# yml-bit/CTA-GAN

Measured on AMD Instinct MI355X. Metric: paired 512x512 slices/sec (G+D step); generator rel-L2 vs CPU reference, higher is better.
Workload: dtype bf16; 1 GPU; HdGan stage-2 full G+D train step (G, Reg, STN, D_m, losses, Adam x3), 16 paired 512x512 slices/GPU; per_gpu_batch=16, global_batch=16, size=512, parallelism=single, rccl_ranks=1, dp_backend=none

## Files before the change

### cta_gan_amd/csrc/conv_halo.h

```cpp
#pragma once
#include <stdlib.h>
#include <type_traits>
#include "common.h"
#include "conv_dispatch.h"

struct ConvArgs {
    const void* x;
    const void* w;
    void* y;
    const float* bias;
    int B, Hi, Wi, Cin, x_ld;
    int Ho, Wo, Cout, y_ld;
    int Hs, Ws, oy0, ox0, os, is;
    int frame;
    int pad_mode, act;
    int w_tap_stride;
    int ntaps;
    int taps[64];
    int kh, kw, dy0, dx0;
    float* stats;
    const void* res;
    const void* fold;
    int res_ld, fold_ld;
    const void* bz;
    const float* bmean;
    const float* brstd;
    float* bstats;
    int bz_ld, bact;
    int ncls;
    int s2d;
    int pair_lo;
    unsigned long long* nie_sync;
    int nie_act;
    int nie_budget;
    int c_ntaps[4], c_tap0[4], c_oy0[4], c_ox0[4], c_kh[4], c_kw[4], c_dy0[4], c_dx0[4];
};

typedef const __attribute__((address_space(1))) void* gptr_t;
typedef __attribute__((address_space(3))) void* lptr_t;

extern __device__ __attribute__((aligned(16))) unsigned g_zero_chunk[4];

__device__ __forceinline__ void unpack_bf16x8(const u32x4 t, float (&f)[8]) {
#pragma unroll
    for (int i = 0; i < 4; ++i) {
        f[2 * i] = __uint_as_float(t[i] << 16);
        f[2 * i + 1] = __uint_as_float(t[i] & 0xffff0000u);
    }
}
__device__ __forceinline__ void add_bf16x8(float (&f)[8], const bf16_t* p) {
    const u32x4 t = *reinterpret_cast<const u32x4*>(p);
#pragma unroll
    for (int i = 0; i < 4; ++i) {
        f[2 * i] += __uint_as_float(t[i] << 16);
        f[2 * i + 1] += __uint_as_float(t[i] & 0xffff0000u);
    }
}

#define HALO_W 16

template <typename T, typename OutT, int BN, int WM, int WN, int KCH, int ABUF, int TH, bool FUSE, int KWC, bool MC = false, bool PK = false,
          bool S2D = false, bool NIE = false>
__global__ __launch_bounds__(WM * WN * 64, ((TH / WM) * (BN / (WN * 16)) > 16 ? 2 : 4))
void conv_halo_kernel(const ConvArgs a) {
    static_assert(!NIE || (!MC && !S2D && sizeof(T) == 2 && !std::is_same<OutT, float>::value),
                  "InstanceNorm in the epilogue: plain bf16 / split-pair launches");
    static_assert(!S2D || (!MC && !FUSE && KWC == 0 && ABUF == 1), "polyphase K walk: plain single-buffer instantiations");
    static_assert(!PK || (KCH == 8 && sizeof(T) == 2), "split-pair K steps: [hi 32 | lo 32] rows of bf16");
    constexpr int NTH = WM * WN * 64;
    constexpr int EPC = VecOf<T>::N;
    constexpr int BKE = KCH * EPC;
    constexpr int BM = TH * HALO_W;
    constexpr int TM = TH / WM;
    static_assert(TH % WM == 0, "tile rows per wave");
    constexpr int TN = BN / (WN * 16);
    constexpr int B_CH = BN * KCH;
    constexpr int B_IT = (B_CH + NTH - 1) / NTH;
    static_assert(B_CH % 64 == 0, "weight tile");
    extern __shared__ __attribute__((aligned(16))) char smem[];

    const int tid = threadIdx.x, lane = tid & 63, wave = __builtin_amdgcn_readfirstlane(tid >> 6);
    const int wm = wave / WN, wn = wave % WN;
    const int n = blockIdx.y;
// ... 8 lines not shown
        kh_ = a.c_kh[q]; kw_ = a.c_kw[q]; dy0 = a.c_dy0[q]; dx0 = a.c_dx0[q];
        ntaps = a.c_ntaps[q]; tap0 = a.c_tap0[q]; oy0_ = a.c_oy0[q]; ox0_ = a.c_ox0[q];
    }
    const int HPW = KWC ? HALO_W + KWC - 1 : HALO_W + kw_ - 1, HPH = TH + kh_ - 1;
    const int HPC = HPH * HPW * KCH;
    const int HPC64 = (HPC + 63) & ~63;
    const int nchunk = a.Cin / BKE;
    const int nbufA = (nchunk > 1 && ABUF == 2) ? 2 : 1;
    char* sA = smem;
    char* sB = smem + nbufA * HPC64 * 16;

    const int tx_n = (a.Ws + HALO_W - 1) / HALO_W;
    const int y0 = (sp / tx_n) * TH, x0 = (sp % tx_n) * HALO_W;
    const T* __restrict__ X = (const T*)a.x + (size_t)n * a.Hi * a.Wi * a.x_ld;
    const T* __restrict__ W = (const T*)a.w;

    const int h_it = (HPC64 + NTH - 1) / NTH;
    const unsigned hpw_magic = (unsigned)((0x100000000ULL + HPW - 1) / HPW);
    const int Hi = a.Hi, Wi = a.Wi, x_ld = a.x_ld, pad_mode = a.pad_mode;
    const int iy00 = y0 + dy0, ix00 = x0 + dx0;
    constexpr bool PRE = (KWC >= 3) && !MC;
    constexpr int H_PRE = PRE ? ((((TH + KWC - 1) * (HALO_W + KWC - 1) * KCH + 63) & ~63) + NTH - 1) / NTH : 1;
    int hoff[H_PRE];
    if constexpr (PRE) {
#pragma unroll
        for (int it = 0; it < H_PRE; ++it) {
            const int sl = tid + NTH * it;
            const int hrow = sl / KCH;
            const int hy = (int)__umulhi((unsigned)hrow, hpw_magic), hx = hrow - hy * HPW;
            const int kc = swz<KCH>(hx, sl % KCH);
// ... 110 lines not shown
#pragma unroll
            for (int mt = 0; mt < TM; ++mt)
#pragma unroll
                for (int nt = 0; nt < TN; ++nt) {
                    if constexpr (sizeof(T) == 2) {
                        acc[mt][nt] = __builtin_amdgcn_mfma_f32_16x16x32_bf16(
                            __builtin_bit_cast(bf16x8, fb[nt]), __builtin_bit_cast(bf16x8, fa[mt]), acc[mt][nt], 0, 0, 0);
                    } else {
                        const f32x4 va = __builtin_bit_cast(f32x4, fa[mt]);
                        const f32x4 vb = __builtin_bit_cast(f32x4, fb[nt]);
#pragma unroll
                        for (int q = 0; q < 4; ++q)
                            acc[mt][nt] = __builtin_amdgcn_mfma_f32_16x16x4f32(vb[q], va[q], acc[mt][nt], 0, 0, 0);
                    }
                }
        }
    };

    const bool wave_rows_valid = y0 + wm * TM < a.Hs;
    const int pps = (h_it + ntaps - 1) / ntaps;
    auto issue_halo_all = [&](int buf, int kc0) __attribute__((always_inline)) {
        if constexpr (PRE) {
#pragma unroll
            for (int j = 0; j < H_PRE; ++j)
                if (NTH * j + 64 * wave < HPC64) {
                    const T* src = hoff[j] >= 0 ? X + (hoff[j] + kc0) : (const T*)g_zero_chunk;
                    __builtin_amdgcn_global_load_lds((gptr_t)src, (lptr_t)(sA + (buf * HPC64 + NTH * j + 64 * wave) * 16), 16, 0, 0);
                }
        } else {
            for (int it = 0; it < h_it; ++it) issue_halo(it, buf, kc0);
// ... 369 lines not shown
        __syncthreads();
#pragma unroll
        for (int it = 0; it < NIT; ++it) {
            const int cidx = tid + NTH * it;
            const int prow = cidx / CPR, ch = (cidx % CPR) * 8;
            const int oy = y0 + prow / HALO_W, ox = x0 + prow % HALO_W;
            if (oy < a.Hs && ox < a.Ws && n0 + ch < a.Cout) {
                OutT* yp = Y + (((size_t)n * a.Ho + (oy * a.os + oy0_)) * a.Wo + (ox * a.os + ox0_)) * a.y_ld + n0 + ch;
                u32x4 v = *reinterpret_cast<const u32x4*>(st + prow * RS + ch * 2);
                if constexpr (FUSE) {
                    float f[8], g[8];
                    unpack_bf16x8(v, f);
                    unpack_bf16x8(rv[it], g);
#pragma unroll
                    for (int e = 0; e < 8; ++e) f[e] += g[e];
                    if (F != nullptr) {
                        const int ey = oy == 1 ? 0 : (oy == a.Hs - 2 ? a.Hs + 1 : -1);
                        const int ex = ox == 1 ? 0 : (ox == a.Ws - 2 ? a.Ws + 1 : -1);
                        const OutT* Fn = F + (size_t)n * (a.Hs + 2) * (a.Ws + 2) * a.fold_ld + n0 + ch;
                        if (ey >= 0) add_bf16x8(f, Fn + ((size_t)ey * (a.Ws + 2) + ox + 1) * a.fold_ld);
                        if (ex >= 0) add_bf16x8(f, Fn + ((size_t)(oy + 1) * (a.Ws + 2) + ex) * a.fold_ld);
                        if (ey >= 0 && ex >= 0) add_bf16x8(f, Fn + ((size_t)ey * (a.Ws + 2) + ex) * a.fold_ld);
                    }
                    bf16x8 o;
#pragma unroll
                    for (int e = 0; e < 8; ++e) o[e] = (bf16_t)f[e];
                    v = __builtin_bit_cast(u32x4, o);
                    if (bst) {
                        float zf[8];
                        unpack_bf16x8(zv[it], zf);
// ... 71 lines not shown
                    }
                }
                if (vec_ok) {
                    *reinterpret_cast<f32x4*>(yp + co) = f32x4{v[0], v[1], v[2], v[3]};
                } else {
#pragma unroll
                    for (int r = 0; r < 4; ++r)
                        if (co + r < a.Cout) yp[co + r] = v[r];
                }
            }
        }
    }
}

template <typename T, typename OutT, int BN, int WM, int WN, int KCH, int ABUF, int TH = 16, bool FUSE = false, int KWC = 0, bool MC = false, bool PK = false,
          bool S2D = false, bool NIE = false>
static int launch_halo_cfg(const ConvArgs& a, hipStream_t st, int* tiles_out = nullptr) {
    if constexpr (!NIE && KWC == 3 && (TH == 16 || (TH == 8 && !PK)) && BN == 128 && WM == 4 && WN == 2 && KCH == 8 && !MC && !S2D &&
                  sizeof(T) == 2 && ((std::is_same<OutT, bf16_t>::value && !PK) || (std::is_same<OutT, bfpair_t>::value && PK))) {
        if (a.nie_sync != nullptr) {
            if ((FUSE && (a.fold != nullptr || a.bstats != nullptr)) || a.stats == nullptr || a.Cout % BN) return CTG_EINVAL;
            return launch_halo_cfg<T, OutT, BN, WM, WN, KCH, ABUF, TH, FUSE, KWC, false, PK, false, true>(a, st, tiles_out);
        }
    }
    if constexpr (!S2D && !FUSE && !MC && KWC == 0 && TH == 16 && sizeof(T) == 2 && KCH == 8 && BN >= 64 && !std::is_same<OutT, float>::value) {
        if (a.s2d) {
            if (a.res != nullptr || a.fold != nullptr) return -1;
            return launch_halo_cfg<T, OutT, BN, WM, WN, KCH, ABUF, TH, false, 0, false, PK, true>(a, st, tiles_out);
        }
    }
    if (a.s2d && !S2D) return -1;
    if constexpr (!FUSE && !MC && !S2D && !NIE) {
        if (a.res != nullptr || a.fold != nullptr) return launch_halo_cfg<T, OutT, BN, WM, WN, KCH, ABUF, TH, true, KWC, false, PK>(a, st, tiles_out);
    }
    if constexpr (!MC && !S2D && !FUSE && KWC == 0 && (TH == 16 || (TH == 8 && BN == 64)) && sizeof(T) == 2 &&
                  ((std::is_same<OutT, bf16_t>::value && !PK) || (std::is_same<OutT, bfpair_t>::value && PK))) {
        if (a.ncls == 4) return launch_halo_cfg<T, OutT, BN, WM, WN, KCH, ABUF, TH, false, 0, true, PK>(a, st, tiles_out);
    }
    if constexpr (KWC == 0 && !MC && !S2D && sizeof(T) == 2) {
        if (a.kw == 3 && a.kh <= 3 && a.ncls <= 1) return launch_halo_cfg<T, OutT, BN, WM, WN, KCH, ABUF, TH, FUSE, 3, false, PK>(a, st, tiles_out);
    }
    if (a.ncls > 1 && !MC && !S2D) return -1;
    if (a.nie_sync != nullptr && !NIE) return CTG_EINVAL;
    constexpr int NTH = WM * WN * 64;
    const int hpw = HALO_W + a.kw - 1, hph = TH + a.kh - 1;
    const int hpc = hph * hpw * KCH;
    const int hpc64 = (hpc + 63) & ~63;
    const int epc = VecOf<T>::N;
    const int nchunk = a.Cin / (KCH * epc);
    const int main_lds = (((nchunk > 1 && ABUF == 2) ? 2 : 1) * hpc64 + 2 * BN * KCH) * 16;
    const int epi_lds = std::is_same<OutT, bfpair_t>::value ? TH * HALO_W * ((BN / WN) * 4 + 16)
                        : sizeof(OutT) == 2 ? TH * HALO_W * (BN * 2 + 16) : 0;
    if (FUSE && a.bstats != nullptr && WM * WN * 64 * 64 > (main_lds > epi_lds ? main_lds : epi_lds)) return -1;
    const int smem = main_lds > epi_lds ? main_lds : epi_lds;
    if (smem > 160 * 1024 || hph * hpw >= 65536) return -1;
    static unsigned long long attr_mask = 0;
    {
        const int rc = ctg_lds_attr_once((const void*)conv_halo_kernel<T, OutT, BN, WM, WN, KCH, ABUF, TH, FUSE, KWC, MC, PK, S2D, NIE>,
                                         160 * 1024, &attr_mask);
        if (rc != CTG_OK) return rc;
    }
    const int tiles = ((a.Hs + TH - 1) / TH) * ((a.Ws + HALO_W - 1) / HALO_W) * (MC ? 4 : 1);
    if (tiles_out != nullptr) *tiles_out = tiles;
    const int ntn = (a.Cout + BN - 1) / BN;
    if constexpr (NIE) {
        static int occ_dev[64];
        int dev = 0;
        if (hipGetDevice(&dev) != hipSuccess) dev = 0;
        dev &= 63;
        if (occ_dev[dev] == 0) {
            int occ = 0;
            if (hipOccupancyMaxActiveBlocksPerMultiprocessor(
                    &occ, (const void*)conv_halo_kernel<T, OutT, BN, WM, WN, KCH, ABUF, TH, FUSE, KWC, MC, PK, S2D, NIE>, NTH, smem) != hipSuccess ||
                occ < 1)
                occ = 1;
            occ_dev[dev] = occ;
        }
        const int share = ctg_knobs().nie_share > 0 ? ctg_knobs().nie_share : 2;
        if ((long)tiles * ntn * share > (long)occ_dev[dev] * ctg_cu_count()) return 2;
    }
    dim3 grid(tiles * ntn, a.B);
    hipLaunchKernelGGL((conv_halo_kernel<T, OutT, BN, WM, WN, KCH, ABUF, TH, FUSE, KWC, MC, PK, S2D, NIE>), grid, dim3(NTH), smem, st, a);
    return ctg_launch_status();
}

static int launch_strip32(const ConvArgs& a, hipStream_t st, int* tiles_out, bool pair);

template <typename T, int KCH>
static int launch_halo_t(const ConvArgs& a, int out_f32, hipStream_t st, int* tiles_out) {
    if (a.is != 1 && !a.s2d) return -1;
    if (out_f32 >= 2) {
        if constexpr (sizeof(T) == 2 && KCH == 8) {
            if (out_f32 == 2) {
                if (a.Cout > 64) return launch_halo_cfg<T, bfpair_t, 128, 4, 2, 8, 1, 16, false, 0, false, true>(a, st, tiles_out);
                if (a.Cout > 32) {
                    if (a.ncls == 4 && !ctg_knobs().no_mc_th8) return launch_halo_cfg<T, bfpair_t, 64, 4, 1, 8, 1, 8, false, 0, false, true>(a, st, tiles_out);
                    if (!ctg_knobs().no_th8_64 && a.ncls <= 1 && a.Hs >= 16)
// ... 53 lines not shown
```

### cta_gan_amd/csrc/conv_igemm.hip

```cpp
#include <stdlib.h>
#include "conv_halo.h"
#include "conv_strip.h"
#include "conv_stript.h"
#include "conv_pair_strips.h"
#include "conv_strips2.h"
#include "conv_strips2w.h"

__device__ __attribute__((aligned(16))) unsigned g_zero_chunk[4];

#ifndef CTG_BIG_TILE
#define CTG_BIG_TILE 1
#endif
static inline int gather_bm(bool bf16, bool k8, int omode, int Cout, long pixels) {
    return (bf16 && k8 && omode == 0 && Cout > 64 && pixels >= 4096 && CTG_BIG_TILE && !ctg_knobs().no_big_tile) ? 256 : 128;
}

#define FRAME_EDGE_PAD 128
__device__ __forceinline__ void grid_pixel(const ConvArgs& a, int m, int& j, int& i) {
    if (a.frame) {
        const int l1 = a.Hs - 2;
        const int p0 = (a.Ws + FRAME_EDGE_PAD - 1) & ~(FRAME_EDGE_PAD - 1), p1 = (l1 + FRAME_EDGE_PAD - 1) & ~(FRAME_EDGE_PAD - 1);
        if (m < p0) { j = 0; i = m < a.Ws ? m : a.Ws - 1; }
        else if (m < 2 * p0) { j = a.Hs - 1; i = m - p0 < a.Ws ? m - p0 : a.Ws - 1; }
        else {
// ... 473 lines not shown
        return launch_cfg<T, T, 128, 32, 4, 1, KCH, 2>(a, st);
    }
    if (out_f32 || sizeof(T) == 4) return launch_cfg<T, float, 128, 16, 4, 1, KCH, 2>(a, st);
    return CTG_EINVAL;
}

extern "C" int ctg_conv_igemm(int dtype, int out_f32, const void* x, const void* w, void* y, const float* bias,
                              int B, int Hi, int Wi, int Cin, int x_ld, int Ho, int Wo, int Cout, int y_ld,
                              int Hs, int Ws, int oy0, int ox0, int os, int is, int frame, int pad_mode, int act,
                              int w_npad, int ntaps, const int* taps_host, float* stats_part, int* stats_slabs_out,
                              const ctg_conv_epilogue* epi, void* stream) {
    CTG_ENTER();
    const void* res = epi ? epi->res : nullptr;
    const void* fold = epi ? epi->fold : nullptr;
    const int res_ld = epi ? epi->res_ld : 0, fold_ld = epi ? epi->fold_ld : 0;
    if (ntaps < 1 || ntaps > 64 || B < 1 || Hs < 1 || Ws < 1 || Cout < 1) return CTG_EINVAL;
    if (frame != 0 && (frame != 1 || Hs < 3 || Ws < 3)) return CTG_EINVAL;
    if (frame != 0 && stats_part != nullptr) return CTG_EINVAL;
    if (dtype != DT_F32 && dtype != DT_BF16 && dtype != DT_PAIR) return CTG_EINVAL;
    const bool pair = dtype == DT_PAIR;
    if (pair) {
        if (x_ld % 16 != 0 || x_ld < 2 * Cin || Cin % 32 != 0 || (out_f32 != 0 && out_f32 != 1)) return CTG_EINVAL;
        if (!out_f32 && (y_ld % 16 != 0 || y_ld < 2 * Cout || Cout % 8 != 0 || ((uintptr_t)y & 15))) return CTG_EINVAL;
        dtype = DT_BF16;
    } else if (out_f32 != 0 && out_f32 != 1) return CTG_EINVAL;
    const int omode = pair ? (out_f32 ? 3 : 2) : out_f32;
    const int epc = dtype == DT_BF16 ? 8 : 4;
    if (Cin % (4 * epc) != 0 || x_ld % epc != 0 || x_ld < Cin || y_ld < Cout) return CTG_EINVAL;
    if (((uintptr_t)x & 15) || ((uintptr_t)w & 15)) return CTG_EINVAL;
    const bool narrow_out = out_f32 || dtype == DT_F32;
    if (!narrow_out && (Cout % 8 != 0 || y_ld % 8 != 0 || ((uintptr_t)y & 15))) return CTG_EINVAL;
    const int bn = Cout > 64 ? 128 : Cout > 32 ? 64 : Cout > 16 ? 32 : 16;
    if (w_npad < ((Cout + bn - 1) / bn) * bn) return CTG_EINVAL;
    if ((Hs - 1) * os + oy0 >= Ho || (Ws - 1) * os + ox0 >= Wo) return CTG_EINVAL;
    if (stats_slabs_out != nullptr) *stats_slabs_out = 0;
    const bool fused = res != nullptr || fold != nullptr;
    if (fused) {
        if (os != 1 || is != 1 || frame || oy0 || ox0 || Ho != Hs || Wo != Ws || Hs < 4 || Ws < 4 || (out_f32 && Cout <= 16)) return CTG_EINVAL;
        if (res != nullptr && (res_ld < Cout || res_ld % epc || ((uintptr_t)res & 15))) return CTG_EINVAL;
        if (fold != nullptr && (fold_ld < Cout || fold_ld % epc || ((uintptr_t)fold & 15))) return CTG_EINVAL;
    }
    ConvArgs a;
    a.stats = nullptr;
    a.ncls = 1;
    a.nie_sync = nullptr; a.nie_act = ACT_NONE; a.nie_budget = 0;
    a.res = res; a.fold = fold; a.res_ld = res_ld; a.fold_ld = fold_ld;
    a.bz = nullptr; a.bmean = nullptr; a.brstd = nullptr; a.bstats = nullptr; a.bz_ld = 0; a.bact = ACT_NONE;
    if (epi != nullptr && epi->bstats != nullptr) {
        if (!fused || dtype != DT_BF16 || (pair && out_f32) || epi->bz == nullptr || epi->bmean == nullptr || epi->brstd == nullptr ||
            epi->bz_ld < Cout || epi->bz_ld % 8 || ((uintptr_t)epi->bz & 15) || Cout <= 16) return CTG_EINVAL;
        if (epi->bact != ACT_NONE && epi->bact != ACT_RELU && epi->bact != ACT_LRELU) return CTG_EINVAL;
        a.bz = epi->bz; a.bmean = epi->bmean; a.brstd = epi->brstd; a.bstats = epi->bstats; a.bz_ld = epi->bz_ld;
        a.bact = epi->bact;
    }
    a.x = x; a.w = w; a.y = y; a.bias = bias;
    a.B = B; a.Hi = Hi; a.Wi = Wi; a.Cin = Cin; a.x_ld = x_ld;
    a.Ho = Ho; a.Wo = Wo; a.Cout = Cout; a.y_ld = y_ld;
    a.Hs = Hs; a.Ws = Ws; a.oy0 = oy0; a.ox0 = ox0; a.os = os; a.is = is; a.frame = frame;
    a.pad_mode = pad_mode; a.act = act; a.w_tap_stride = w_npad * Cin; a.ntaps = ntaps;
    a.pair_lo = 0;
    const bool k8 = pair || (Cin % (8 * epc)) == 0;
// ... 89 lines not shown
            int ntile = 0;
            const bool want_stats = stats_part != nullptr && stats_slabs_out != nullptr && bias == nullptr &&
                                    act == ACT_NONE && Cout > 16 &&
                                    ((os == 1 && Hs == Ho && Ws == Wo) || os == 2);
            a.stats = want_stats ? stats_part : nullptr;
            int rc = -1;
            if (dtype == DT_BF16) rc = k8 ? launch_halo_t<bf16_t, 8>(a, omode, st, &ntile) : launch_halo_t<bf16_t, 4>(a, omode, st, &ntile);
            else rc = k8 ? launch_halo_t<float, 8>(a, omode, st, &ntile) : launch_halo_t<float, 4>(a, omode, st, &ntile);
            if (rc != -1) {
                if ((want_stats || a.bstats != nullptr) && rc == 0 && stats_slabs_out != nullptr) *stats_slabs_out = ntile;
                return rc;
            }
            a.stats = nullptr;
        }
    }
    if (fused) return CTG_EINVAL;
    if (dtype == DT_BF16 && !out_f32 && !pair) {
        const bool ws = stats_part != nullptr && stats_slabs_out != nullptr;
        int slabs = 0;
        int rc = launch_strips2(a, ws ? stats_part : nullptr, st, &slabs);
        if (rc == -1) rc = launch_strips2w(a, ws ? stats_part : nullptr, st, &slabs);
        if (rc != -1) {
            if (rc == 0 && ws) *stats_slabs_out = slabs;
            return rc;
        }
    }
    int mtiles = 0;
    if (stats_part != nullptr && stats_slabs_out != nullptr && bias == nullptr && act == ACT_NONE &&
        Cout > 16 && os == 1 && !frame && Hs == Ho && Ws == Wo && oy0 == 0 && ox0 == 0) {
        const int bm = gather_bm(dtype == DT_BF16, k8, omode, Cout, (long)Hs * Ws);
// ... 17 lines not shown
                                      void* stream) {
    CTG_ENTER();
    if (stats_slabs_out != nullptr) *stats_slabs_out = 0;
    if (dtype != DT_BF16 && dtype != DT_PAIR) return 2;
    const bool pair = dtype == DT_PAIR;
    if (B < 1 || Hs < 1 || Ws < 1 || Cout < 1 || cls_ntaps == nullptr || cls_oy0 == nullptr || cls_ox0 == nullptr) return CTG_EINVAL;
    if (Cin % 32 != 0 || x_ld % 8 != 0 || x_ld < Cin || y_ld < Cout || Cout % 8 != 0 || y_ld % 8 != 0) return CTG_EINVAL;
    if (pair && (x_ld % 16 || x_ld < 2 * Cin || y_ld % 16 || y_ld < 2 * Cout)) return CTG_EINVAL;
    if (((uintptr_t)x & 15) || ((uintptr_t)w & 15) || ((uintptr_t)y & 15)) return CTG_EINVAL;
    const int bn = Cout > 64 ? 128 : Cout > 32 ? 64 : Cout > 16 ? 32 : 16;
    if (w_npad < ((Cout + bn - 1) / bn) * bn) return CTG_EINVAL;
    if (ctg_knobs().no_halo || ctg_knobs().no_class_merge || Hs < 16 || Ws < 16 || Cout <= 16 || (long)Hi * Wi * x_ld >= (1L << 31)) return 2;
    ConvArgs a;
    a.stats = nullptr;
    a.nie_sync = nullptr; a.nie_act = ACT_NONE; a.nie_budget = 0;
    a.res = nullptr; a.fold = nullptr; a.res_ld = 0; a.fold_ld = 0;
    a.bz = nullptr; a.bmean = nullptr; a.brstd = nullptr; a.bstats = nullptr; a.bz_ld = 0; a.bact = ACT_NONE;
    a.x = x; a.w = w; a.y = y; a.bias = bias;
    a.B = B; a.Hi = Hi; a.Wi = Wi; a.Cin = Cin; a.x_ld = x_ld;
    a.Ho = Ho; a.Wo = Wo; a.Cout = Cout; a.y_ld = y_ld;
    a.Hs = Hs; a.Ws = Ws; a.oy0 = 0; a.ox0 = 0; a.os = 2; a.is = 1; a.frame = 0;
    a.pad_mode = pad_mode; a.act = act; a.w_tap_stride = w_npad * Cin;
    a.ncls = 4;
    a.s2d = 0;
    a.pair_lo = 0;
    if (pair) {
        a.pair_lo = x_ld / 2;
        a.Cin = 2 * Cin;
        a.w_tap_stride = w_npad * 2 * Cin;
    }
    int t0 = 0, kh_max = 1, kw_max = 1;
// ... 37 lines not shown
```

### cta_gan_amd/csrc/conv_strip.h

```cpp
#pragma once
#include "conv_halo.h"

#define STRIP_R 9
#define STRIP_ROWB 1152

struct StripArgs {
    const bf16_t* x;
    const bf16_t* w;
    bf16_t* y;
    const float* bias;
    float* stats;
    int B, H, W, x_ld, y_ld, w_tap_stride;
    int pad_mode, act;
    int band_rows, nbands, nstrips;
    int widx[9];
    int x_lo, y_lo;
};

__device__ __forceinline__ int strip_swz(int px, int c) { return c ^ ((px >> 1) & 3); }

template <bool FLIP, bool EPI>
__global__ __launch_bounds__(256, 2) void conv_strip32_kernel(const StripArgs a) {
    __shared__ __attribute__((aligned(16))) char ring_all[4][STRIP_R][STRIP_ROWB];
    const int tid = threadIdx.x, lane = tid & 63, wave = __builtin_amdgcn_readfirstlane(tid >> 6);
// ... 339 lines not shown
#pragma unroll
            for (int r = 0; r < 4; ++r) {
                const float t1 = row16_sum_to_lane15(s1[nt][r]), t2 = row16_sum_to_lane15(s2[nt][r]);
                if (p == 15) {
                    const int c = nt * 16 + kg * 4 + r;
                    dst[c * 2] = t1;
                    dst[c * 2 + 1] = t2;
                }
            }
    }
}

static int launch_strip32(const ConvArgs& a, hipStream_t st, int* tiles_out, bool pair) {
    if (ctg_knobs().no_strip || a.Cin != (pair ? 64 : 32) || a.Cout != 32 || a.kh != 3 || a.kw != 3 || a.ntaps != 9 || a.is != 1 || a.os != 1 || a.ncls > 1 ||
        a.oy0 != 0 || a.ox0 != 0 || a.Ho != a.Hs || a.Wo != a.Ws || a.Hi != a.Hs || a.Wi != a.Ws || a.res != nullptr ||
        a.fold != nullptr || a.dy0 != -1 || a.dx0 != -1 || a.act > ACT_LRELU)
        return -1;
    if ((long)a.B * a.Hs * a.Ws < (1L << 20) || a.Hs < 32 || a.Ws < 32 || (a.y_ld & 3) || (a.x_ld & 7)) return -1;
    if (pair && (long)a.Hs * a.Ws * a.x_ld >= (1L << 31)) return -1;
    const bool fwd = taps_3x3(a.taps, false);
    if (!fwd && !taps_3x3(a.taps, true)) return -1;
    StripArgs s;
    s.x = (const bf16_t*)a.x; s.w = (const bf16_t*)a.w; s.y = (bf16_t*)a.y; s.bias = a.bias; s.stats = a.stats;
    s.B = a.B; s.H = a.Hs; s.W = a.Ws; s.x_ld = a.x_ld; s.y_ld = a.y_ld; s.w_tap_stride = a.w_tap_stride;
    s.pad_mode = a.pad_mode; s.act = a.act;
    s.x_lo = a.pair_lo; s.y_lo = a.y_ld / 2;
    s.nstrips = (a.Ws + 15) / 16;
    const BandPlan bp = band_plan(a.Hs, 32, (long)ctg_cu_count() * 4 * (pair ? 2 : 3), (long)a.B * s.nstrips, ctg_knobs().strip_band);
    s.band_rows = bp.band_rows;
    s.nbands = bp.nbands;
    for (int t = 0; t < 9; ++t) s.widx[t] = a.taps[t] >> 16;
// ... 25 lines not shown
```

### cta_gan_amd/engine.py

```python
from __future__ import annotations

import os

from dataclasses import dataclass
from typing import Callable, List, Optional

import torch

from . import dp, ops
from .ops import ACT_LRELU, ACT_NONE, ACT_RELU, ACT_SIGMOID, ACT_TANH, PAD_REFLECT, PAD_ZERO, pack_tap


class Act:
    __slots__ = ("t", "grad", "req", "moments", "in_src", "in_plain", "grad_stats")

    def __init__(self, t: torch.Tensor, req: bool = False):
        self.t = t
        self.grad = None
        self.req = req
        self.moments = None
        self.in_src = None
        self.in_plain = False
        self.grad_stats = None

# ... 388 lines not shown
                weight.detach()[0].flip(-1, -2).reshape(cin, kk).contiguous(), _pack_dtype(dtype), 1, cin, kk, _round_up(cin, 32), 64,
                kk, 1, 0))
        dxp = ops.empty_act((bsz, hi + 2 * p, wi + 2 * p, cin), dtype, dev)
        ops.conv_smallcin(g.reshape(bsz, ho, wo), None, spec.k, 1, 2 * p, PAD_ZERO, wflip, _round_up(cin, 32), None,
                          ACT_NONE, dxp, cin, kxw=kxw)
        add_grad(x, dxp, p)
        return
    wb, npad = _pack_bwd(cache, spec, weight, dtype, kpad=m_c if spec.out_f32 else None)
    if spec.transposed:
        dx = ops.empty_act((bsz, hi, wi, cin), dtype, dev)
        taps = [pack_tap(ky - spec.pad, kx - spec.pad, ky * spec.k + kx) for ky in range(spec.k) for kx in range(spec.k)]
        ops.conv_igemm(gm, wb, npad, dx, None, cin, hi, wi, 0, 0, 1, 2, PAD_ZERO, ACT_NONE, taps)
        add_grad(x, dx, 0)
    elif spec.reflect:
        p = spec.pad
        dxp = ops.empty_act((bsz, hi + 2 * p, wi + 2 * p, cin), dtype, dev)
        assert spec.stride == 1
        taps = [pack_tap(-ky, -kx, ky * spec.k + kx) for ky in range(spec.k) for kx in range(spec.k)]
        if p == 1 and hi % 16 == 0 and wi % 16 == 0 and hi >= 32 and wi >= 32 and not _NO_FRAME:
            taps_in = [pack_tap(p - ky, p - kx, ky * spec.k + kx) for ky in range(spec.k) for kx in range(spec.k)]
            if ops.conv_fusable(cin, hi, wi):
                ops.conv_igemm(gm, wb, npad, dxp, None, cin, hi + 2 * p, wi + 2 * p, 0, 0, 1, 1, PAD_ZERO, ACT_NONE, taps,
                               frame=True)
                res = None
                if x.grad is not None and x.grad[1] == 0 and x.grad[0].dtype == dtype \
                        and tuple(x.grad[0].shape) == (bsz, hi, wi, cin):
                    res, x.grad = x.grad[0], None
                dx = ops.empty_act((bsz, hi, wi, cin), dtype, dev)
                want_in = (x.in_src is not None and x.grad is None and dtype == torch.bfloat16 and not _NO_IN_FUSE)
                in_arg = x.in_src if want_in else None
                if want_in and ops.PAIR_BWD_ACTIVE:
                    zact = x.in_src[3]
                    if zact == ACT_RELU and x.in_plain:
                        in_arg = (x.t, _unit_stats(x.t, 0.0), _unit_stats(x.t, 1.0), ACT_RELU)
                    elif zact != ACT_NONE:
                        want_in, in_arg = False, None
                part, slabs = ops.conv_igemm(gm, wb, npad, dx, None, cin, hi, wi, 0, 0, 1, 1, PAD_ZERO, ACT_NONE, taps_in,
                                             res=res, fold=dxp, in_bwd=in_arg)
                add_grad(x, dx, 0)
                if want_in and slabs > 0:
                    x.grad_stats = (dx, part)
                return
            ops.conv_igemm(gm, wb, npad, dxp, None, cin, hi, wi, p, p, 1, 1, PAD_ZERO, ACT_NONE, taps_in)
            ops.conv_igemm(gm, wb, npad, dxp, None, cin, hi + 2 * p, wi + 2 * p, 0, 0, 1, 1, PAD_ZERO, ACT_NONE, taps,
                           frame=True)
        else:
            ops.conv_igemm(gm, wb, npad, dxp, None, cin, hi + 2 * p, wi + 2 * p, 0, 0, 1, 1, PAD_ZERO, ACT_NONE, taps)
        add_grad(x, dxp, p)
    else:
        dx = ops.empty_act((bsz, hi, wi, cin), dtype, dev)
        _bwd_data_launch(spec, gm, wb, npad, dx, hi, wi, cin)
        add_grad(x, dx, 0)


_UNIT_STATS = {}


def _unit_stats(t, value):
    key = (t.device, t.shape[0], t.shape[3], value)
    hit = _UNIT_STATS.get(key)
    if hit is None:
# ... 224 lines not shown
```

### cta_gan_amd/ops.py

```python
from __future__ import annotations

import ctypes
import os
import threading
from typing import Optional, Sequence

import torch

from . import _lib

ACT_NONE, ACT_RELU, ACT_LRELU, ACT_TANH, ACT_SIGMOID = 0, 1, 2, 3, 4
PAD_ZERO, PAD_REFLECT = 0, 1
_DT = {torch.float32: 0, torch.bfloat16: 1}
_EPC = {torch.float32: 4, torch.bfloat16: 8}


def dt(dtype) -> int:
    return _DT[dtype]


def epc(dtype) -> int:
    return _EPC[dtype]


DT_PAIR = 2
DT_MIX = 3

_env = os.environ.get
_NO_NIE = bool(_env("CTG_NO_NIE"))
NIE_POISON = bool(_env("CTG_NIE_POISON"))
NIE_MAX_WGS = int(_env("CTG_NIE_MAX_WGS", "1024"))
NIE_MAX_WGS_PAIR = int(_env("CTG_NIE_MAX_WGS_PAIR", "2048"))
NIE_BUDGET = int(_env("CTG_NIE_BUDGET", "0"))
NIE_SHARE = max(1, int(_env("CTG_NIE_SHARE", "2") or 2))
_TH8_WGS = 0 if _env("CTG_NO_TH8") is not None else int(_env("CTG_TH8_WGS", "384"))
_NO_HALO = bool(_env("CTG_NO_HALO"))
_NO_EPI_FUSE = bool(_env("CTG_NO_EPI_FUSE"))
_NO_WG_GROUPS_FIX = bool(_env("CTG_NO_WG_GROUPS_FIX"))
_WG_S2_FIX = not _env("CTG_NO_WG_S2_FIX")
_WG_FIX_BELOW = int(_env("CTG_WG_FIX_BELOW", "512"))
_NO_SMALLB = bool(_env("CTG_NO_SMALLB"))
_FIN_FUSE = bool(_env("CTG_FIN_FUSE"))
_NO_KXW = bool(_env("CTG_NO_KXW"))
DETERMINISTIC = bool(_env("CTG_DETERMINISTIC"))


def dtc(t) -> int:
    if _pair_now() and t.dtype == torch.bfloat16:
        return DT_PAIR
    return _DT[t.dtype]


# ... 198 lines not shown


def pack_tap(dy: int, dx: int, widx: int) -> int:
    assert -64 <= dy < 64 and -64 <= dx < 64 and 0 <= widx < 256
    return (dy + 64) | ((dx + 64) << 8) | (widx << 16)


def _tap_array(taps: Sequence[int]):
    return (ctypes.c_int * len(taps))(*taps)


class ConvEpilogue(ctypes.Structure):
    _fields_ = [("res", ctypes.c_void_p), ("fold", ctypes.c_void_p), ("bz", ctypes.c_void_p), ("bmean", ctypes.c_void_p),
                ("brstd", ctypes.c_void_p), ("bstats", ctypes.c_void_p), ("res_ld", ctypes.c_int), ("fold_ld", ctypes.c_int),
                ("bz_ld", ctypes.c_int), ("bact", ctypes.c_int), ("nie_sync", ctypes.c_void_p), ("nie_act", ctypes.c_int),
                ("nie_tiles", ctypes.c_int), ("nie_groups", ctypes.c_int), ("nie_budget", ctypes.c_int)]


_NIE_SYNC = {}
NIE_GROUPS = 4096
NIE_SLOTS = 512


def _nie_sync(device, tiles):
    cap = torch.cuda.is_current_stream_capturing()
    key = (device.index, "graph" if cap else torch.cuda.current_stream(device).cuda_stream, tiles)
    buf = _NIE_SYNC.get(key)
    if buf is None and not cap:
        buf = _NIE_SYNC[key] = torch.zeros(1 + NIE_GROUPS, dtype=torch.int64, device=device)
    return buf

# ... 64 lines not shown
        and _nie_sync(x.device, tiles) is not None


def _nie_tiles(x, cout, hs, ws):
    tiles = ((hs + 15) // 16) * ((ws + 15) // 16)
    if not is_pair(x) and tiles * ((cout + 127) // 128) * x.shape[0] < _TH8_WGS:
        tiles = moments_slabs(hs, ws)
    return tiles


def moments_slabs(hs, ws):
    return ((hs + 7) // 8) * ((ws + 15) // 16)


def conv_igemm(x, w_packed, w_npad, y, bias, cout, hs, ws, oy0, ox0, os_, is_, pad_mode, act, taps, want_stats=False,
               frame=False, res=None, fold=None, in_bwd=None, in_fuse=None):
    lib = _lib.load()
    b, hi, wi, cin, x_ld = _nhwc(x)
    cin0 = cin
    pair_in = is_pair(x)
    if pair_in:
        assert w_packed.dtype == torch.float32 and cin % 32 == 0
        w_packed = split_w_pair(w_packed, cin)
    b2, ho, wo, cy, y_ld = _nhwc(y)
    res_ld = fold_ld = 0
    if res is not None:
        rb, rh, rw, rc, res_ld = _nhwc(res)
        assert (rb, rh, rw, rc) == (b, hs, ws, cout) and res.dtype == y.dtype
    if fold is not None:
        fb, fh, fw, fc, fold_ld = _nhwc(fold)
        assert (fb, fh, fw, fc) == (b, hs + 2, ws + 2, cout) and fold.dtype == y.dtype
# ... 8 lines not shown
    if KERNEL_EVENTS is not None and cin0 == 256 and cout == 256 and len(taps) == 9 and not frame and os_ == 1 and is_ == 1:
        tkey = "fwd_in" if in_fuse is not None else "fwd" if (res is None and fold is None) else "bwd_data"
    part, slabs = None, ctypes.c_int(0)
    if want_stats and bias is None and act == ACT_NONE and cout > 16:
        part = torch.empty(b * moments_slabs(hs, ws) * cout * 2, dtype=torch.float32, device=x.device)
    epi = None
    nie_out = None
    if in_fuse is not None:
        assert part is not None and fold is None and in_bwd is None
        if NIE_POISON:
            part.fill_(float("nan"))
        tiles = _nie_tiles(x, cout, hs, ws)
        nie_out = True
        epi = ConvEpilogue(_p(res), None, None, None, None, None, res_ld, 0, 0, 0, _p(_nie_sync(x.device, tiles)), in_fuse, tiles,
                           NIE_GROUPS, NIE_BUDGET)
    elif res is not None or fold is not None:
        epi = ConvEpilogue(_p(res), _p(fold), None, None, None, None, res_ld, fold_ld, 0, 0, None, 0, 0, 0, 0)
        if in_bwd is not None:
            z, mean, rstd, zact = in_bwd
            zb, zh, zw, zc, z_ld = _nhwc(z)
            assert (zb, zh, zw, zc) == (b, hs, ws, cout) and z.dtype == y.dtype == torch.bfloat16 and not want_stats
            assert is_pair(z) == pair_in
            part = torch.empty(b * moments_slabs(hs, ws) * cout * 2, dtype=torch.float32, device=x.device)
            epi.bz, epi.bmean, epi.brstd, epi.bstats, epi.bz_ld, epi.bact = _p(z), _p(mean), _p(rstd), _p(part), z_ld, zact
    tbytes = None
    if KERNEL_EVENTS is not None and tkey is None and cin0 == 32 and cout == 32 and len(taps) == 9 and not frame \
            and os_ == 1 and is_ == 1 and res is None and fold is None and y.dtype == x.dtype and hs * ws >= 512 * 512:
        tkey = "conv32"
        tbytes = b * hs * ws * (cin0 + cout) * _esz(x) + w_packed.numel() * w_packed.element_size()
    if KERNEL_EVENTS is not None and tkey is None and cin0 == 64 and cout == 128 and len(taps) == 9 and not frame and os_ == 1 \
            and is_ == 2 and res is None and fold is None and y.dtype == x.dtype == torch.bfloat16 and bias is None \
            and hs * ws >= 256 * 256:
        tkey = "convs2"
        tbytes = (x.shape.numel() * _esz(x) + y.shape.numel() * _esz(y)) + w_packed.numel() * w_packed.element_size()
    tok = None
    if OP_LOG is not None:
        npx = (2 * ws + 2 * (hs - 2)) if frame else hs * ws
        nb_ = b * hi * wi * cin0 * _esz(x) + b * npx * cout * _esz(y) * (1 + (res is not None) + (in_bwd is not None)) \
            + len(taps) * cout * cin0 * (4 if pair_in else x.element_size())
        kind = "frame" if frame else "conv+IN" if in_fuse is not None else "fused bwd-data" if (res is not None or fold is not None) else "conv"
        tok = _log_begin("%s %d->%d %dtaps is%d os%d @%dx%d%s" % (kind, cin0, cout, len(taps), is_, os_, hs, ws,
                                                                   " +INsums" if in_bwd is not None else ""),
                         2.0 * b * npx * cout * cin0 * len(taps), nb_)
    e0 = _timed_begin(tkey, tbytes)
    st = lib.ctg_conv_igemm(DT_PAIR if pair_in else dt(x.dtype), out_f32, _p(x), _p(w_packed), _p(y), _p(bias), b, hi, wi, cin, x_ld,
                            ho, wo, cout, y_ld, hs, ws, oy0, ox0, os_, is_, int(frame), pad_mode, act, w_npad, len(taps), arr,
                            _p(part) if in_bwd is None else None, ctypes.addressof(slabs) if part is not None else None,
                            ctypes.addressof(epi) if epi is not None else None, _stream())
    _timed_end(tkey, e0)
    if in_fuse is not None and st == 2:
        _NIE_REFUSED.add((x.device.index, pair_in, b, cin0, cout, hs, ws))
        return None
    _log_end(tok)
    _lib.check(st, "ctg_conv_igemm")
    if in_fuse is not None:
        return nie_out
    if part is not None and slabs.value > 0:
        part = part[:b * slabs.value * cout * 2].view(b, slabs.value, cout, 2)
    return part, slabs.value


def conv_igemm_classes(x, w_packed, w_npad, y, bias, cout, hs, ws, classes, pad_mode, act, want_stats=False):
    if x.dtype != torch.bfloat16 or y.dtype != torch.bfloat16 or len(classes) != 4 or any(not c[2] for c in classes):
        return None
    if hs < 16 or ws < 16 or cout <= 16:
        return None
# ... 1035 lines not shown
```

### include/ctagan_hip.h

```cpp
#ifndef CTAGAN_HIP_H
#define CTAGAN_HIP_H

#ifdef __cplusplus
extern "C" {
#endif

#define CTG_ABI_VERSION 15
int ctg_abi_version(void);

typedef struct ctg_conv_epilogue {
    const void* res;
    const void* fold;
    const void* bz;
    const float* bmean;
    const float* brstd;
    float* bstats;
    int res_ld, fold_ld, bz_ld;
    int bact;
    void* nie_sync;
    int nie_act;
    int nie_tiles;
    int nie_groups;
    int nie_budget;
} ctg_conv_epilogue;

int ctg_conv_igemm(int dtype, int out_f32, const void* x, const void* w, void* y, const float* bias,
                   int B, int Hi, int Wi, int Cin, int x_ld, int Ho, int Wo, int Cout, int y_ld,
                   int Hs, int Ws, int oy0, int ox0, int os, int is, int frame, int pad_mode, int act,
                   int w_npad, int ntaps, const int* taps_host, float* stats_part, int* stats_slabs_out,
                   const ctg_conv_epilogue* epi, void* stream);
int ctg_conv_igemm_classes(int dtype, const void* x, const void* w, void* y, const float* bias, int B, int Hi, int Wi,
                           int Cin, int x_ld, int Ho, int Wo, int Cout, int y_ld, int Hs, int Ws, int pad_mode, int act,
                           int w_npad, const int* cls_ntaps, const int* cls_oy0, const int* cls_ox0, const int* taps,
                           float* stats_part, int* stats_slabs_out, void* stream);

int ctg_conv_wgrad(int dtype, const void* g, const void* x, float* part, int B, int Hs, int Ws, int Mc, int g_ld,
                   int Hi, int Wi, int Nc, int x_ld, int is, int pad_mode, int slab, int ntaps,
                   const int* taps_host, void* stream);
// ... 129 lines not shown
```

Baseline: 339.1 slices/s.

## Fold reflect-pad border gradients into fused 3x3 backward-data conv kernel

Adds an RF template variant of the halo conv kernel. It accumulates the reflect-padding ring contributions straight into the border output rows and columns by issuing extra MFMAs on the mirrored halo rows and columns. This removes the separate frame conv launch, the padded dxp scratch buffer, and the fold read in the epilogue for reflect-padded 3x3 layers. The cost is extra MFMA work and branches on the border tiles. The path refuses (returns 2) for pair inputs, odd shapes, or when occupancy limits are hit, and then falls back to the old two-launch path.

```diff
diff --git a/cta_gan_amd/csrc/conv_halo.h b/cta_gan_amd/csrc/conv_halo.h
--- a/cta_gan_amd/csrc/conv_halo.h
+++ b/cta_gan_amd/csrc/conv_halo.h
@@ -30,6 +30,7 @@
     int ncls;
     int s2d;
     int pair_lo;
+    int rfold;
     unsigned long long* nie_sync;
     int nie_act;
     int nie_budget;
@@ -60,13 +61,15 @@
 #define HALO_W 16
 
 template <typename T, typename OutT, int BN, int WM, int WN, int KCH, int ABUF, int TH, bool FUSE, int KWC, bool MC = false, bool PK = false,
-          bool S2D = false, bool NIE = false>
+          bool S2D = false, bool NIE = false, bool RF = false>
 __global__ __launch_bounds__(WM * WN * 64, ((TH / WM) * (BN / (WN * 16)) > 16 ? 2 : 4))
 void conv_halo_kernel(const ConvArgs a) {
     static_assert(!NIE || (!MC && !S2D && sizeof(T) == 2 && !std::is_same<OutT, float>::value),
                   "InstanceNorm in the epilogue: plain bf16 / split-pair launches");
     static_assert(!S2D || (!MC && !FUSE && KWC == 0 && ABUF == 1), "polyphase K walk: plain single-buffer instantiations");
     static_assert(!PK || (KCH == 8 && sizeof(T) == 2), "split-pair K steps: [hi 32 | lo 32] rows of bf16");
+    static_assert(!RF || (FUSE && KWC == 3 && !MC && !PK && !S2D && !NIE && sizeof(T) == 2 && std::is_same<OutT, T>::value),
+                  "reflect fold: the fused 3x3 bf16 backward-data launches");
     constexpr int NTH = WM * WN * 64;
     constexpr int EPC = VecOf<T>::N;
     constexpr int BKE = KCH * EPC;
@@ -105,6 +108,14 @@
     const int y0 = (sp / tx_n) * TH, x0 = (sp % tx_n) * HALO_W;
     const T* __restrict__ X = (const T*)a.x + (size_t)n * a.Hi * a.Wi * a.x_ld;
     const T* __restrict__ W = (const T*)a.w;
+    int rf_top = -1, rf_bot = -1;
+    bool rf_left = false, rf_right = false;
+    if constexpr (RF) {
+        if (y0 == 0 && wm == 1 / TM) rf_top = 1 % TM;
+        if (y0 + TH == a.Hs && wm == (TH - 2) / TM) rf_bot = (TH - 2) % TM;
+        rf_left = x0 == 0;
+        rf_right = x0 + HALO_W == a.Ws;
+    }
 
     const int h_it = (HPC64 + NTH - 1) / NTH;
     const unsigned hpw_magic = (unsigned)((0x100000000ULL + HPW - 1) / HPW);
@@ -245,6 +256,50 @@
                             acc[mt][nt] = __builtin_amdgcn_mfma_f32_16x16x4f32(vb[q], va[q], acc[mt][nt], 0, 0, 0);
                     }
                 }
+            if constexpr (RF) {
+                const int rsh = ky == 2 ? -2 : 2;
+                const int mrow = ky == 2 ? rf_top : ky == 0 ? rf_bot : -1;
+                const bool mcol = (kx == 2 && rf_left) || (kx == 0 && rf_right);
+                if (mrow >= 0) {
+#pragma unroll
+                    for (int mt = 0; mt < TM; ++mt)
+                        if (mt == mrow) {
+                            const u32x4 fr = *reinterpret_cast<const u32x4*>(prow + xo + (mt + rsh) * (HPW * KCH * 16));
+#pragma unroll
+                            for (int nt = 0; nt < TN; ++nt)
+                                acc[mt][nt] = __builtin_amdgcn_mfma_f32_16x16x32_bf16(
+                                    __builtin_bit_cast(bf16x8, fb[nt]), __builtin_bit_cast(bf16x8, fr), acc[mt][nt], 0, 0, 0);
+                        }
+                }
+                if (mcol) {
+                    const int hxm = kx == 2 ? hx - 2 : hx + 2;
+                    const int xc = ((hxm * KCH + swz<KCH>(hxm, lane >> 4)) * 16) ^ (ks * 64);
+                    const bool mine = (lane & 15) == (kx == 2 ? 1 : HALO_W - 2);
+#pragma unroll
+                    for (int mt = 0; mt < TM; ++mt) {
+                        u32x4 fc = *reinterpret_cast<const u32x4*>(prow + xc + mt * (HPW * KCH * 16));
+#pragma unroll
+                        for (int q = 0; q < 4; ++q) fc[q] = mine ? fc[q] : 0u;
+#pragma unroll
+                        for (int nt = 0; nt < TN; ++nt)
+                            acc[mt][nt] = __builtin_amdgcn_mfma_f32_16x16x32_bf16(
+                                __builtin_bit_cast(bf16x8, fb[nt]), __builtin_bit_cast(bf16x8, fc), acc[mt][nt], 0, 0, 0);
+                    }
+                    if (mrow >= 0) {
+#pragma unroll
+                        for (int mt = 0; mt < TM; ++mt)
+                            if (mt == mrow) {
+                                u32x4 fc = *reinterpret_cast<const u32x4*>(prow + xc + (mt + rsh) * (HPW * KCH * 16));
+#pragma unroll
+                                for (int q = 0; q < 4; ++q) fc[q] = mine ? fc[q] : 0u;
+#pragma unroll
+                                for (int nt = 0; nt < TN; ++nt)
+                                    acc[mt][nt] = __builtin_amdgcn_mfma_f32_16x16x32_bf16(
+                                        __builtin_bit_cast(bf16x8, fb[nt]), __builtin_bit_cast(bf16x8, fc), acc[mt][nt], 0, 0, 0);
+                            }
+                    }
+                }
+            }
         }
     };
 
@@ -644,6 +699,7 @@
                     unpack_bf16x8(rv[it], g);
 #pragma unroll
                     for (int e = 0; e < 8; ++e) f[e] += g[e];
+                    if constexpr (!RF)
                     if (F != nullptr) {
                         const int ey = oy == 1 ? 0 : (oy == a.Hs - 2 ? a.Hs + 1 : -1);
                         const int ex = ox == 1 ? 0 : (ox == a.Ws - 2 ? a.Ws + 1 : -1);
@@ -745,7 +801,7 @@
 }
 
 template <typename T, typename OutT, int BN, int WM, int WN, int KCH, int ABUF, int TH = 16, bool FUSE = false, int KWC = 0, bool MC = false, bool PK = false,
-          bool S2D = false, bool NIE = false>
+          bool S2D = false, bool NIE = false, bool RF = false>
 static int launch_halo_cfg(const ConvArgs& a, hipStream_t st, int* tiles_out = nullptr) {
     if constexpr (!NIE && KWC == 3 && (TH == 16 || (TH == 8 && !PK)) && BN == 128 && WM == 4 && WN == 2 && KCH == 8 && !MC && !S2D &&
                   sizeof(T) == 2 && ((std::is_same<OutT, bf16_t>::value && !PK) || (std::is_same<OutT, bfpair_t>::value && PK))) {
@@ -762,7 +818,8 @@
     }
     if (a.s2d && !S2D) return -1;
     if constexpr (!FUSE && !MC && !S2D && !NIE) {
-        if (a.res != nullptr || a.fold != nullptr) return launch_halo_cfg<T, OutT, BN, WM, WN, KCH, ABUF, TH, true, KWC, false, PK>(a, st, tiles_out);
+        if (a.res != nullptr || a.fold != nullptr || a.rfold)
+            return launch_halo_cfg<T, OutT, BN, WM, WN, KCH, ABUF, TH, true, KWC, false, PK>(a, st, tiles_out);
     }
     if constexpr (!MC && !S2D && !FUSE && KWC == 0 && (TH == 16 || (TH == 8 && BN == 64)) && sizeof(T) == 2 &&
                   ((std::is_same<OutT, bf16_t>::value && !PK) || (std::is_same<OutT, bfpair_t>::value && PK))) {
@@ -770,6 +827,17 @@
     }
     if constexpr (KWC == 0 && !MC && !S2D && sizeof(T) == 2) {
         if (a.kw == 3 && a.kh <= 3 && a.ncls <= 1) return launch_halo_cfg<T, OutT, BN, WM, WN, KCH, ABUF, TH, FUSE, 3, false, PK>(a, st, tiles_out);
+    }
+    if constexpr (!RF) {
+        if (a.rfold) {
+            if constexpr (FUSE && KWC == 3 && !MC && !PK && !S2D && !NIE && sizeof(T) == 2 && std::is_same<OutT, T>::value &&
+                          !(BN == 64 && KCH == 8 && TH == 16)) {
+                if (a.fold != nullptr || a.kh != 3 || a.dy0 != -1 || a.dx0 != -1 || a.Hs % TH || a.Ws % HALO_W) return 2;
+                return launch_halo_cfg<T, OutT, BN, WM, WN, KCH, ABUF, TH, true, 3, false, false, false, false, true>(a, st, tiles_out);
+            } else {
+                return 2;
+            }
+        }
     }
     if (a.ncls > 1 && !MC && !S2D) return -1;
     if (a.nie_sync != nullptr && !NIE) return CTG_EINVAL;
@@ -787,7 +855,7 @@
     if (smem > 160 * 1024 || hph * hpw >= 65536) return -1;
     static unsigned long long attr_mask = 0;
     {
-        const int rc = ctg_lds_attr_once((const void*)conv_halo_kernel<T, OutT, BN, WM, WN, KCH, ABUF, TH, FUSE, KWC, MC, PK, S2D, NIE>,
+        const int rc = ctg_lds_attr_once((const void*)conv_halo_kernel<T, OutT, BN, WM, WN, KCH, ABUF, TH, FUSE, KWC, MC, PK, S2D, NIE, RF>,
                                          160 * 1024, &attr_mask);
         if (rc != CTG_OK) return rc;
     }
@@ -802,7 +870,7 @@
         if (occ_dev[dev] == 0) {
             int occ = 0;
             if (hipOccupancyMaxActiveBlocksPerMultiprocessor(
-                    &occ, (const void*)conv_halo_kernel<T, OutT, BN, WM, WN, KCH, ABUF, TH, FUSE, KWC, MC, PK, S2D, NIE>, NTH, smem) != hipSuccess ||
+                    &occ, (const void*)conv_halo_kernel<T, OutT, BN, WM, WN, KCH, ABUF, TH, FUSE, KWC, MC, PK, S2D, NIE, RF>, NTH, smem) != hipSuccess ||
                 occ < 1)
                 occ = 1;
             occ_dev[dev] = occ;
@@ -811,7 +879,7 @@
         if ((long)tiles * ntn * share > (long)occ_dev[dev] * ctg_cu_count()) return 2;
     }
     dim3 grid(tiles * ntn, a.B);
-    hipLaunchKernelGGL((conv_halo_kernel<T, OutT, BN, WM, WN, KCH, ABUF, TH, FUSE, KWC, MC, PK, S2D, NIE>), grid, dim3(NTH), smem, st, a);
+    hipLaunchKernelGGL((conv_halo_kernel<T, OutT, BN, WM, WN, KCH, ABUF, TH, FUSE, KWC, MC, PK, S2D, NIE, RF>), grid, dim3(NTH), smem, st, a);
     return ctg_launch_status();
 }
 
diff --git a/cta_gan_amd/csrc/conv_igemm.hip b/cta_gan_amd/csrc/conv_igemm.hip
--- a/cta_gan_amd/csrc/conv_igemm.hip
+++ b/cta_gan_amd/csrc/conv_igemm.hip
@@ -511,6 +511,7 @@
     const void* res = epi ? epi->res : nullptr;
     const void* fold = epi ? epi->fold : nullptr;
     const int res_ld = epi ? epi->res_ld : 0, fold_ld = epi ? epi->fold_ld : 0;
+    const bool rfold = epi != nullptr && epi->rfold != 0;
     if (ntaps < 1 || ntaps > 64 || B < 1 || Hs < 1 || Ws < 1 || Cout < 1) return CTG_EINVAL;
     if (frame != 0 && (frame != 1 || Hs < 3 || Ws < 3)) return CTG_EINVAL;
     if (frame != 0 && stats_part != nullptr) return CTG_EINVAL;
@@ -531,7 +532,23 @@
     if (w_npad < ((Cout + bn - 1) / bn) * bn) return CTG_EINVAL;
     if ((Hs - 1) * os + oy0 >= Ho || (Ws - 1) * os + ox0 >= Wo) return CTG_EINVAL;
     if (stats_slabs_out != nullptr) *stats_slabs_out = 0;
-    const bool fused = res != nullptr || fold != nullptr;
+    const bool fused = res != nullptr || fold != nullptr || rfold;
+    if (rfold) {
+        if (fold != nullptr || epi->nie_sync != nullptr) return CTG_EINVAL;
+        bool ok = !ctg_knobs().no_halo && dtype == DT_BF16 && !out_f32 && ntaps == 9 && os == 1 && is == 1 && !frame && oy0 == 0 && ox0 == 0 &&
+                  Ho == Hs && Wo == Ws && Hi == Hs && Wi == Ws && pad_mode == PAD_ZERO && bias == nullptr && act == ACT_NONE &&
+                  Hs % 16 == 0 && Ws % 16 == 0 && Hs >= 32 && Ws >= 32 && Cout > 16 && (long)Hi * Wi * x_ld < (1L << 31);
+        if (ok) {
+            unsigned seen = 0;
+            for (int t = 0; t < ntaps; ++t) {
+                const int dy = tap_dy(taps_host[t]), dx = tap_dx(taps_host[t]);
+                if (dy < -1 || dy > 1 || dx < -1 || dx > 1) { ok = false; break; }
+                seen |= 1u << ((dy + 1) * 3 + dx + 1);
+            }
+            ok = ok && seen == 0x1ffu;
+        }
+        if (!ok) return 2;
+    }
     if (fused) {
         if (os != 1 || is != 1 || frame || oy0 || ox0 || Ho != Hs || Wo != Ws || Hs < 4 || Ws < 4 || (out_f32 && Cout <= 16)) return CTG_EINVAL;
         if (res != nullptr && (res_ld < Cout || res_ld % epc || ((uintptr_t)res & 15))) return CTG_EINVAL;
@@ -541,7 +558,7 @@
     a.stats = nullptr;
     a.ncls = 1;
     a.nie_sync = nullptr; a.nie_act = ACT_NONE; a.nie_budget = 0;
-    a.res = res; a.fold = fold; a.res_ld = res_ld; a.fold_ld = fold_ld;
+    a.res = res; a.fold = fold; a.res_ld = res_ld; a.fold_ld = fold_ld; a.rfold = rfold ? 1 : 0;
     a.bz = nullptr; a.bmean = nullptr; a.brstd = nullptr; a.bstats = nullptr; a.bz_ld = 0; a.bact = ACT_NONE;
     if (epi != nullptr && epi->bstats != nullptr) {
         if (!fused || dtype != DT_BF16 || (pair && out_f32) || epi->bz == nullptr || epi->bmean == nullptr || epi->brstd == nullptr ||
@@ -661,6 +678,7 @@
             a.stats = nullptr;
         }
     }
+    if (rfold) return 2;
     if (fused) return CTG_EINVAL;
     if (dtype == DT_BF16 && !out_f32 && !pair) {
         const bool ws = stats_part != nullptr && stats_slabs_out != nullptr;
@@ -708,7 +726,7 @@
     ConvArgs a;
     a.stats = nullptr;
     a.nie_sync = nullptr; a.nie_act = ACT_NONE; a.nie_budget = 0;
-    a.res = nullptr; a.fold = nullptr; a.res_ld = 0; a.fold_ld = 0;
+    a.res = nullptr; a.fold = nullptr; a.res_ld = 0; a.fold_ld = 0; a.rfold = 0;
     a.bz = nullptr; a.bmean = nullptr; a.brstd = nullptr; a.bstats = nullptr; a.bz_ld = 0; a.bact = ACT_NONE;
     a.x = x; a.w = w; a.y = y; a.bias = bias;
     a.B = B; a.Hi = Hi; a.Wi = Wi; a.Cin = Cin; a.x_ld = x_ld;
diff --git a/cta_gan_amd/csrc/conv_strip.h b/cta_gan_amd/csrc/conv_strip.h
--- a/cta_gan_amd/csrc/conv_strip.h
+++ b/cta_gan_amd/csrc/conv_strip.h
@@ -377,7 +377,7 @@
 static int launch_strip32(const ConvArgs& a, hipStream_t st, int* tiles_out, bool pair) {
     if (ctg_knobs().no_strip || a.Cin != (pair ? 64 : 32) || a.Cout != 32 || a.kh != 3 || a.kw != 3 || a.ntaps != 9 || a.is != 1 || a.os != 1 || a.ncls > 1 ||
         a.oy0 != 0 || a.ox0 != 0 || a.Ho != a.Hs || a.Wo != a.Ws || a.Hi != a.Hs || a.Wi != a.Ws || a.res != nullptr ||
-        a.fold != nullptr || a.dy0 != -1 || a.dx0 != -1 || a.act > ACT_LRELU)
+        a.fold != nullptr || a.rfold || a.dy0 != -1 || a.dx0 != -1 || a.act > ACT_LRELU)
         return -1;
     if ((long)a.B * a.Hs * a.Ws < (1L << 20) || a.Hs < 32 || a.Ws < 32 || (a.y_ld & 3) || (a.x_ld & 7)) return -1;
     if (pair && (long)a.Hs * a.Ws * a.x_ld >= (1L << 31)) return -1;
diff --git a/cta_gan_amd/engine.py b/cta_gan_amd/engine.py
--- a/cta_gan_amd/engine.py
+++ b/cta_gan_amd/engine.py
@@ -426,14 +426,11 @@
         add_grad(x, dx, 0)
     elif spec.reflect:
         p = spec.pad
-        dxp = ops.empty_act((bsz, hi + 2 * p, wi + 2 * p, cin), dtype, dev)
         assert spec.stride == 1
         taps = [pack_tap(-ky, -kx, ky * spec.k + kx) for ky in range(spec.k) for kx in range(spec.k)]
         if p == 1 and hi % 16 == 0 and wi % 16 == 0 and hi >= 32 and wi >= 32 and not _NO_FRAME:
             taps_in = [pack_tap(p - ky, p - kx, ky * spec.k + kx) for ky in range(spec.k) for kx in range(spec.k)]
             if ops.conv_fusable(cin, hi, wi):
-                ops.conv_igemm(gm, wb, npad, dxp, None, cin, hi + 2 * p, wi + 2 * p, 0, 0, 1, 1, PAD_ZERO, ACT_NONE, taps,
-                               frame=True)
                 res = None
                 if x.grad is not None and x.grad[1] == 0 and x.grad[0].dtype == dtype \
                         and tuple(x.grad[0].shape) == (bsz, hi, wi, cin):
@@ -447,16 +444,27 @@
                         in_arg = (x.t, _unit_stats(x.t, 0.0), _unit_stats(x.t, 1.0), ACT_RELU)
                     elif zact != ACT_NONE:
                         want_in, in_arg = False, None
-                part, slabs = ops.conv_igemm(gm, wb, npad, dx, None, cin, hi, wi, 0, 0, 1, 1, PAD_ZERO, ACT_NONE, taps_in,
-                                             res=res, fold=dxp, in_bwd=in_arg)
+                out = None
+                if not ops.NO_RFOLD and not ops.is_pair(gm):
+                    out = ops.conv_igemm(gm, wb, npad, dx, None, cin, hi, wi, 0, 0, 1, 1, PAD_ZERO, ACT_NONE, taps_in,
+                                         res=res, in_bwd=in_arg, rfold=True)
+                if out is None:
+                    dxp = ops.empty_act((bsz, hi + 2 * p, wi + 2 * p, cin), dtype, dev)
+                    ops.conv_igemm(gm, wb, npad, dxp, None, cin, hi + 2 * p, wi + 2 * p, 0, 0, 1, 1, PAD_ZERO, ACT_NONE, taps,
+                                   frame=True)
+                    out = ops.conv_igemm(gm, wb, npad, dx, None, cin, hi, wi, 0, 0, 1, 1, PAD_ZERO, ACT_NONE, taps_in,
+                                         res=res, fold=dxp, in_bwd=in_arg)
+                part, slabs = out
                 add_grad(x, dx, 0)
                 if want_in and slabs > 0:
                     x.grad_stats = (dx, part)
                 return
+            dxp = ops.empty_act((bsz, hi + 2 * p, wi + 2 * p, cin), dtype, dev)
             ops.conv_igemm(gm, wb, npad, dxp, None, cin, hi, wi, p, p, 1, 1, PAD_ZERO, ACT_NONE, taps_in)
             ops.conv_igemm(gm, wb, npad, dxp, None, cin, hi + 2 * p, wi + 2 * p, 0, 0, 1, 1, PAD_ZERO, ACT_NONE, taps,
                            frame=True)
         else:
+            dxp = ops.empty_act((bsz, hi + 2 * p, wi + 2 * p, cin), dtype, dev)
             ops.conv_igemm(gm, wb, npad, dxp, None, cin, hi + 2 * p, wi + 2 * p, 0, 0, 1, 1, PAD_ZERO, ACT_NONE, taps)
         add_grad(x, dxp, p)
     else:
diff --git a/cta_gan_amd/ops.py b/cta_gan_amd/ops.py
--- a/cta_gan_amd/ops.py
+++ b/cta_gan_amd/ops.py
@@ -36,6 +36,7 @@
 _TH8_WGS = 0 if _env("CTG_NO_TH8") is not None else int(_env("CTG_TH8_WGS", "384"))
 _NO_HALO = bool(_env("CTG_NO_HALO"))
 _NO_EPI_FUSE = bool(_env("CTG_NO_EPI_FUSE"))
+NO_RFOLD = bool(_env("CTG_NO_RFOLD"))
 _NO_WG_GROUPS_FIX = bool(_env("CTG_NO_WG_GROUPS_FIX"))
 _WG_S2_FIX = not _env("CTG_NO_WG_S2_FIX")
 _WG_FIX_BELOW = int(_env("CTG_WG_FIX_BELOW", "512"))
@@ -264,7 +265,7 @@
     _fields_ = [("res", ctypes.c_void_p), ("fold", ctypes.c_void_p), ("bz", ctypes.c_void_p), ("bmean", ctypes.c_void_p),
                 ("brstd", ctypes.c_void_p), ("bstats", ctypes.c_void_p), ("res_ld", ctypes.c_int), ("fold_ld", ctypes.c_int),
                 ("bz_ld", ctypes.c_int), ("bact", ctypes.c_int), ("nie_sync", ctypes.c_void_p), ("nie_act", ctypes.c_int),
-                ("nie_tiles", ctypes.c_int), ("nie_groups", ctypes.c_int), ("nie_budget", ctypes.c_int)]
+                ("nie_tiles", ctypes.c_int), ("nie_groups", ctypes.c_int), ("nie_budget", ctypes.c_int), ("rfold", ctypes.c_int)]
 
 
 _NIE_SYNC = {}
@@ -359,7 +360,7 @@
 
 
 def conv_igemm(x, w_packed, w_npad, y, bias, cout, hs, ws, oy0, ox0, os_, is_, pad_mode, act, taps, want_stats=False,
-               frame=False, res=None, fold=None, in_bwd=None, in_fuse=None):
+               frame=False, res=None, fold=None, in_bwd=None, in_fuse=None, rfold=False):
     lib = _lib.load()
     b, hi, wi, cin, x_ld = _nhwc(x)
     cin0 = cin
@@ -398,8 +399,8 @@
         nie_out = True
         epi = ConvEpilogue(_p(res), None, None, None, None, None, res_ld, 0, 0, 0, _p(_nie_sync(x.device, tiles)), in_fuse, tiles,
                            NIE_GROUPS, NIE_BUDGET)
-    elif res is not None or fold is not None:
-        epi = ConvEpilogue(_p(res), _p(fold), None, None, None, None, res_ld, fold_ld, 0, 0, None, 0, 0, 0, 0)
+    elif res is not None or fold is not None or rfold:
+        epi = ConvEpilogue(_p(res), _p(fold), None, None, None, None, res_ld, fold_ld, 0, 0, None, 0, 0, 0, 0, int(bool(rfold)))
         if in_bwd is not None:
             z, mean, rstd, zact = in_bwd
             zb, zh, zw, zc, z_ld = _nhwc(z)
@@ -422,10 +423,15 @@
         npx = (2 * ws + 2 * (hs - 2)) if frame else hs * ws
         nb_ = b * hi * wi * cin0 * _esz(x) + b * npx * cout * _esz(y) * (1 + (res is not None) + (in_bwd is not None)) \
             + len(taps) * cout * cin0 * (4 if pair_in else x.element_size())
-        kind = "frame" if frame else "conv+IN" if in_fuse is not None else "fused bwd-data" if (res is not None or fold is not None) else "conv"
-        tok = _log_begin("%s %d->%d %dtaps is%d os%d @%dx%d%s" % (kind, cin0, cout, len(taps), is_, os_, hs, ws,
-                                                                   " +INsums" if in_bwd is not None else ""),
-                         2.0 * b * npx * cout * cin0 * len(taps), nb_)
+        kind = "frame" if frame else "conv+IN" if in_fuse is not None else "fused bwd-data" if (res is not None or fold is not None or rfold) \
+            else "conv"
+        flop = 2.0 * b * npx * cout * cin0 * len(taps)
+        if rfold:
+            flop += 2.0 * b * cout * cin0 * (3 * (2 * ws + 2 * hs) + 4)
+        tok = _log_begin("%s %d->%d %dtaps is%d os%d @%dx%d%s%s" % (kind, cin0, cout, len(taps), is_, os_, hs, ws,
+                                                                     " +ring" if rfold else "",
+                                                                     " +INsums" if in_bwd is not None else ""),
+                         flop, nb_)
     e0 = _timed_begin(tkey, tbytes)
     st = lib.ctg_conv_igemm(DT_PAIR if pair_in else dt(x.dtype), out_f32, _p(x), _p(w_packed), _p(y), _p(bias), b, hi, wi, cin, x_ld,
                             ho, wo, cout, y_ld, hs, ws, oy0, ox0, os_, is_, int(frame), pad_mode, act, w_npad, len(taps), arr,
@@ -434,6 +440,8 @@
     _timed_end(tkey, e0)
     if in_fuse is not None and st == 2:
         _NIE_REFUSED.add((x.device.index, pair_in, b, cin0, cout, hs, ws))
+        return None
+    if rfold and st == 2:
         return None
     _log_end(tok)
     _lib.check(st, "ctg_conv_igemm")
diff --git a/include/ctagan_hip.h b/include/ctagan_hip.h
--- a/include/ctagan_hip.h
+++ b/include/ctagan_hip.h
@@ -22,6 +22,7 @@
     int nie_tiles;
     int nie_groups;
     int nie_budget;
+    int rfold;
 } ctg_conv_epilogue;
 
 int ctg_conv_igemm(int dtype, int out_f32, const void* x, const void* w, void* y, const float* bias,
```

After: 337.8 slices/s. About the same (-0.4%).
